# abcqmars/audio-visual-sepatation-in-visual-agnostic-situtation

Measured on AMD Instinct MI355X. Metric: mixtures/sec (train step, 2-src MUSIC shape), higher is better.
Workload: dtype f32; 1 GPU; full HIP path, AV train step: 2-source mix, batch 64/GPU (BASELINE configs[2] shape), 65535-sample waveforms -> HIP STFT 1022/256 -> 256x256 log-freq tiles, 3x224^2 frames/source, unet7+hidsep(sig)+resnet18dilated, BCE, SGD; f32 arithmetic; visual trunk on this library (no MIOpen kernel in the step); global_batch=64, parallelism=dp1

## Files before the change

### audio-visual-sepatation-in-visual-agnostic-situtation_amd/csrc/ops.hip

```cpp
#include "common.h"
#include "warp_coords.h"
#include <string.h>
#include <stdio.h>

__global__ __launch_bounds__(256) void channel_stats_kernel(const float* __restrict__ x, int N, int C, int HW,
                                                            double* __restrict__ stats) {
  const int c = blockIdx.x;
  const long long total = (long long)N * HW;
  const long long per = (total + gridDim.y - 1) / gridDim.y;
  const long long beg = per * blockIdx.y, end = min(total, beg + per);
  float s = 0.f, q = 0.f;
  double ds = 0.0, dq = 0.0;
  int cnt = 0;
  for (long long i = beg + threadIdx.x; i < end; i += 256) {
    int n = (int)(i / HW), hw = (int)(i % HW);
    float v = x[((long long)n * C + c) * HW + hw];
    s += v;
    q += v * v;
    if (++cnt == 64) { ds += s; dq += q; s = q = 0.f; cnt = 0; }
  }
  ds += s;
  dq += q;
  block_stats_add(ds, dq, c, C, stats);
}
// ... 857 lines not shown
      for (int s = 0; s < S; ++s) {
        float d = 1.f;
        if (act == AVSEP_ACT_SIGMOID) d = p[s] * (1.f - p[s]);
        else if (act == AVSEP_ACT_TANH) d = 1.f - p[s] * p[s];
        else if (act == AVSEP_ACT_RELU) d = l[s] > 0.f ? 1.f : 0.f;
        dlogits[((long long)b * S + s) * FT + i] = g[s] * d;
      }
    }
  }
}

extern "C" int avsep_mask_loss_bwd(const float* logits, const float* gt, const float* weight, int64_t w_target_stride,
                                   const float* coef, int32_t B, int32_t S, int32_t FT, int32_t act, int32_t loss,
                                   float* dlogits, avsep_stream_t stream) {
  if (!logits || !gt || !coef || !dlogits || B <= 0 || B > 65535 || S < 1 || S > MAXS || FT <= 0) return AVSEP_ERR_ARG;
  if (loss < 0 || loss > 2) return AVSEP_ERR_ARG;
  int gx = min(cdiv(FT, 1024), 64);
  hipLaunchKernelGGL(mask_loss_bwd_kernel, dim3(gx, B), dim3(256), 0, (hipStream_t)stream, logits, gt, weight,
                     (long long)w_target_stride, coef, B, S, FT, act, loss, dlogits);
  AVSEP_LAUNCH_CHECK();
  return AVSEP_OK;
}

__global__ __launch_bounds__(256) void maxpool_fwd_kernel(const float* __restrict__ x, const float* __restrict__ scale,
                                                          const float* __restrict__ shift, int act, int C, int NC, int H,
                                                          int W, int Ho, int Wo, float* __restrict__ y,
                                                          int* __restrict__ idx) {
  const long long total = (long long)NC * Ho * Wo;
  for (long long i = (long long)blockIdx.x * 256 + threadIdx.x; i < total; i += (long long)gridDim.x * 256) {
    int wo = (int)(i % Wo), ho = (int)((i / Wo) % Ho);
    long long nc = i / ((long long)Wo * Ho);
    const int c = (int)(nc % C);
    const float sc = scale ? scale[c] : 1.f, sh = scale ? shift[c] : 0.f;
    const float* p = x + nc * H * W;
    float best = -INFINITY;
    int bi = -1;
    for (int kh = 0; kh < 3; ++kh) {
      int h = ho * 2 - 1 + kh;
      if ((unsigned)h >= (unsigned)H) continue;
      for (int kw = 0; kw < 3; ++kw) {
        int w = wo * 2 - 1 + kw;
        if ((unsigned)w >= (unsigned)W) continue;
        float v = act_apply(fmaf(p[h * W + w], sc, sh), act);
        if (v > best || bi < 0) { best = v; bi = h * W + w; }
      }
    }
    y[i] = best;
    if (idx) idx[i] = bi;
  }
}
__global__ __launch_bounds__(256) void maxpool_fwd4_kernel(const float* __restrict__ x, const float* __restrict__ scale,
                                                           const float* __restrict__ shift, int act, int C, int H, int W,
                                                           int Ho, int Wo, float* __restrict__ y, int* __restrict__ idx) {
  const int nc = blockIdx.y, c = nc % C, Wq = Wo >> 2;
  const int t = blockIdx.x * 256 + threadIdx.x;
  if (t >= Ho * Wq) return;
  const int ho = t / Wq, q = t - ho * Wq;
  const float sc = scale ? scale[c] : 1.f, sh = scale ? shift[c] : 0.f, slope = act_slope(act);
  const float* p = x + (long long)nc * H * W;
  float best[4] = {-INFINITY, -INFINITY, -INFINITY, -INFINITY};
  int bi[4] = {-1, -1, -1, -1};
#pragma unroll
  for (int kh = 0; kh < 3; ++kh) {
    const int h = 2 * ho - 1 + kh;
    if ((unsigned)h >= (unsigned)H) continue;
    const float* row = p + h * W + 8 * q;
    const f32x4 a = *reinterpret_cast<const f32x4*>(row), b = *reinterpret_cast<const f32x4*>(row + 4);
    float v[9];
    v[0] = q > 0 ? row[-1] : 0.f;
    v[1] = a.x; v[2] = a.y; v[3] = a.z; v[4] = a.w; v[5] = b.x; v[6] = b.y; v[7] = b.z; v[8] = b.w;
#pragma unroll
    for (int k = 0; k < 9; ++k) v[k] = act_by_slope(fmaf(v[k], sc, sh), slope);
#pragma unroll
    for (int j = 0; j < 4; ++j)
#pragma unroll
      for (int kw = 0; kw < 3; ++kw) {
        const int k = 2 * j + kw;
        if (k == 0 && q == 0) continue;
        if (v[k] > best[j] || bi[j] < 0) { best[j] = v[k]; bi[j] = h * W + 8 * q - 1 + k; }
      }
  }
  const long long o = ((long long)nc * Ho + ho) * Wo + 4 * q;
  *reinterpret_cast<f32x4*>(y + o) = f32x4{best[0], best[1], best[2], best[3]};
  if (idx) *reinterpret_cast<int4*>(idx + o) = make_int4(bi[0], bi[1], bi[2], bi[3]);
}

enum { MAXPOOL_FWD_4, MAXPOOL_FWD_GENERIC };
static GluePlan maxpool_fwd_plan(int C, long long NC, int H, int W) {
  if (NC <= 0 || NC > 0x7fffffffLL || H <= 0 || W <= 0 || C <= 0 || NC % C) return glue_refused();
  int Ho = (H + 2 - 3) / 2 + 1, Wo = (W + 2 - 3) / 2 + 1;
  if ((W & 7) == 0 && (H & 1) == 0 && NC <= 65535 && (long long)H * W < 0x7fffffffLL)
    return GluePlan{MAXPOOL_FWD_4, dim3(cdiv(Ho * (Wo >> 2), 256), (unsigned)NC)};
  long long total = NC * Ho * Wo;
  return GluePlan{MAXPOOL_FWD_GENERIC, dim3((int)min((total + 255) / 256, (long long)65536))};
}
extern "C" int avsep_maxpool3x3s2_fwd(const float* x, const float* scale, const float* shift, int32_t act, int32_t C,
                                      int32_t NC, int32_t H, int32_t W, float* y, int32_t* idx, avsep_stream_t stream) {
  const GluePlan pl = maxpool_fwd_plan(C, NC, H, W);
  if (!x || !y || pl.refused()) return AVSEP_ERR_ARG;
  if ((scale == nullptr) != (shift == nullptr)) return AVSEP_ERR_ARG;
  int Ho = (H + 2 - 3) / 2 + 1, Wo = (W + 2 - 3) / 2 + 1;
  switch (pl.form) {
    case MAXPOOL_FWD_4:
      hipLaunchKernelGGL(maxpool_fwd4_kernel, pl.grid, dim3(256), 0, (hipStream_t)stream, x, scale, shift, act,
                         C, H, W, Ho, Wo, y, idx);
      break;
    case MAXPOOL_FWD_GENERIC:
      hipLaunchKernelGGL(maxpool_fwd_kernel, pl.grid, dim3(256), 0,
                         (hipStream_t)stream, x, scale, shift, act, C, NC, H, W, Ho, Wo, y, idx);
      break;
  }
  AVSEP_LAUNCH_CHECK();
  return AVSEP_OK;
}

__global__ __launch_bounds__(256) void maxpool_bwd_kernel(const float* __restrict__ dy, const int* __restrict__ idx, int NC,
                                                          int H, int W, int Ho, int Wo, float* __restrict__ dx) {
  const long long total = (long long)NC * H * W;
  for (long long i = (long long)blockIdx.x * 256 + threadIdx.x; i < total; i += (long long)gridDim.x * 256) {
    int w = (int)(i % W), h = (int)((i / W) % H);
    long long nc = i / ((long long)W * H);
    int self = h * W + w;
    float s = 0.f;
    for (int ho = h / 2; ho <= (h + 1) / 2 && ho < Ho; ++ho)
      for (int wo = w / 2; wo <= (w + 1) / 2 && wo < Wo; ++wo) {
        long long o = (nc * Ho + ho) * Wo + wo;
        if (idx[o] == self) s += dy[o];
      }
    dx[i] = s;
  }
}
static GluePlan maxpool_bwd_plan(long long NC, int H, int W) {
  if (NC <= 0 || NC > 0x7fffffffLL || H <= 0 || W <= 0) return glue_refused();
  long long total = NC * H * W;
  return GluePlan{0, dim3((int)min((total + 255) / 256, (long long)65536))};
}
// ... 191 lines not shown
                                               const float* shift, const float* pqr, int32_t N, int32_t C, int32_t H, int32_t W,
                                               float* dy, avsep_stream_t stream) {
  const GluePlan pl = maxpool_bn_relu_bwd_apply_plan(N, C, H, W);
  if (!g || !idx || !y || !scale || !shift || !pqr || !dy || pl.refused()) return AVSEP_ERR_ARG;
  const int Ho = (H + 2 - 3) / 2 + 1, Wo = (W + 2 - 3) / 2 + 1;
  switch (pl.form) {
    case POOL_BWD_APPLY_4:
      hipLaunchKernelGGL(maxpool_bn_relu_bwd_apply4_kernel, pl.grid, dim3(256), 0, (hipStream_t)stream, g, idx, y, scale,
                         shift, pqr, C, H, W, Ho, Wo, dy);
      break;
    case POOL_BWD_APPLY_PAIR:
      hipLaunchKernelGGL(maxpool_bn_relu_bwd_apply_kernel, pl.grid, dim3(256), 0, (hipStream_t)stream, g, idx, y, scale,
                         shift, pqr, C, H, W, Ho, Wo, dy);
      break;
    case POOL_BWD_APPLY_1:
      hipLaunchKernelGGL(maxpool_bn_relu_bwd_apply1_kernel, pl.grid, dim3(256), 0,
                         (hipStream_t)stream, g, idx, y, scale, shift, pqr, C, N * C, H, W, Ho, Wo, dy);
      break;
  }
  AVSEP_LAUNCH_CHECK();
  return AVSEP_OK;
}

__global__ __launch_bounds__(256) void temporal_mean_fwd_kernel(const float* __restrict__ x, int B, int T, long long CHW,
                                                                float* __restrict__ y) {
  const long long total = (long long)B * CHW;
  for (long long i = (long long)blockIdx.x * 256 + threadIdx.x; i < total; i += (long long)gridDim.x * 256) {
    long long b = i / CHW, r = i % CHW;
    float s = 0.f;
    for (int t = 0; t < T; ++t) s += x[(b * T + t) * CHW + r];
    y[i] = s / (float)T;
  }
}
static GluePlan flat_plan(long long total, long long cap) {
  return GluePlan{0, dim3((int)min((total + 255) / 256, cap))};
}
static GluePlan temporal_mean_plan(int B, int T, long long CHW, bool bwd) {
  if (B <= 0 || T <= 0 || CHW <= 0 || CHW > 0x7fffffffLL) return glue_refused();
  return flat_plan(bwd ? (long long)B * T * CHW : (long long)B * CHW, 65536);
}
extern "C" int avsep_temporal_mean_fwd(const float* x, int32_t B, int32_t T, int32_t CHW, float* y,
                                       avsep_stream_t stream) {
  const GluePlan pl = temporal_mean_plan(B, T, CHW, false);
  if (!x || !y || pl.refused()) return AVSEP_ERR_ARG;
  hipLaunchKernelGGL(temporal_mean_fwd_kernel, pl.grid, dim3(256), 0,
                     (hipStream_t)stream, x, B, T, (long long)CHW, y);
// ... 183 lines not shown
    atomicAdd(&sums[r * 3 + 2], sh[8] + sh[9] + sh[10] + sh[11]);
  }
}
extern "C" int avsep_sdr_sums(const float* est, const float* ref, int32_t R, int32_t L, int64_t est_stride,
                              int64_t ref_stride, double* sums, avsep_stream_t stream) {
  if (!est || !ref || !sums || R <= 0 || R > 65535 || L <= 0) return AVSEP_ERR_ARG;
  hipLaunchKernelGGL(sdr_sums_kernel, dim3(min(cdiv(L, 2048), 64), R), dim3(256), 0, (hipStream_t)stream, est, ref, L,
                     (long long)est_stride, (long long)ref_stride, sums);
  AVSEP_LAUNCH_CHECK();
  return AVSEP_OK;
}

static const GluePlanRow ops_glue_rows[] = {
    {"channel_stats", {"chunks"}, [](int N, int C, int H, int W, int) { return channel_stats_plan(N, C, (long long)H * W); }},
    {"bn_bwd_apply", {"vec4", "scalar"}, [](int N, int C, int H, int W, int) { return bn_bwd_apply_plan(N, C, (long long)H * W); }},
    {"affine_act", {"vec4", "scalar"}, [](int N, int C, int H, int W, int) { return affine_act_plan(N, C, (long long)H * W); }},
    {"affine_act_bwd", {"v4", "v1"}, [](int N, int C, int H, int W, int) { return affine_act_bwd_plan(N, C, (long long)H * W); }},
    {"relu_up2x_fwd", {"pair", "fwd4", "generic"}, [](int N, int C, int H, int W, int aux) { return relu_up2x_fwd_plan(N, C, H, W, aux != 0); }},
    {"relu_up2x_bwd", {"sweep,planes", "sweep", "tile"}, [](int N, int C, int H, int W, int aux) { return relu_up2x_bwd_plan(N, C, H, W, aux != 0); }},
    {"maxpool_fwd", {"fwd4", "generic"}, [](int N, int C, int H, int W, int) { return maxpool_fwd_plan(C, (long long)N * C, H, W); }},
    {"maxpool_bwd", {"gather"}, [](int N, int C, int H, int W, int) { return maxpool_bwd_plan((long long)N * C, H, W); }},
    {"maxpool_bn_relu_bwd_stats", {"plane"}, [](int N, int C, int H, int W, int) { return maxpool_bn_relu_bwd_stats_plan(N, C, H, W); }},
    {"maxpool_bn_relu_bwd_apply", {"apply4", "pair", "apply1"}, [](int N, int C, int H, int W, int) { return maxpool_bn_relu_bwd_apply_plan(N, C, H, W); }},
    {"space_to_depth2", {"planes"}, [](int N, int C, int H, int W, int Cp) { return space_to_depth2_plan(N, C, H, W, Cp); }},
    {"temporal_mean_fwd", {"flat"}, [](int B, int C, int H, int W, int T) { return temporal_mean_plan(B, T, (long long)C * H * W, false); }},
    {"temporal_mean_bwd", {"flat"}, [](int B, int C, int H, int W, int T) { return temporal_mean_plan(B, T, (long long)C * H * W, true); }},
    {"sgd", {"flat"}, [](int N, int C, int H, int W, int) { return flat_plan((long long)N * C * ((long long)H * W), 16384); }},
};

extern "C" int avsep_glue_plan(const char* op, int32_t N, int32_t C, int32_t H, int32_t W, int32_t aux, char* form, size_t cap,
                               int32_t grid[3]) {
  if (!op || !form || !grid || cap < 32 || N <= 0 || C <= 0 || H <= 0 || W <= 0 || aux < 0) return AVSEP_ERR_ARG;
  int counts[2] = {(int)(sizeof(ops_glue_rows) / sizeof(ops_glue_rows[0])), 0};
  const GluePlanRow* const tables[2] = {ops_glue_rows, b16_glue_rows(&counts[1])};
  for (int t = 0; t < 2; ++t)
    for (const GluePlanRow* r = tables[t]; r < tables[t] + counts[t]; ++r) {
      if (strcmp(op, r->op)) continue;
      const GluePlan p = r->plan(N, C, H, W, aux);
      if (p.refused()) return AVSEP_ERR_ARG;
      snprintf(form, cap, "%s", r->forms[p.form]);
      grid[0] = (int32_t)p.grid.x; grid[1] = (int32_t)p.grid.y; grid[2] = (int32_t)p.grid.z;
      return AVSEP_OK;
    }
  return AVSEP_ERR_ARG;
}

// ... 12 lines not shown
```

### audio-visual-sepatation-in-visual-agnostic-situtation_amd/kernels.py

```python
import ctypes as C
import os

import numpy as np
import torch

from . import lib
from .lib import ConvDesc, CatDesc, call, ptr


def _f32(shape, like):
    return torch.empty(shape, dtype=torch.float32, device=like.device)


FMT_F32, FMT_B16 = 0, 1


def is_b16(t):
    return t is not None and t.dtype == torch.bfloat16


def fmt_of(t):
    return FMT_B16 if is_b16(t) else FMT_F32


# ... 1235 lines not shown
        g, g2 = to_b16(g), to_b16(g2)
        call("avsep_b16_maxpool_bn_relu_bwd", ptr(g), ptr(g2), ptr(idx), ptr(y), ptr(bnrow[0]), ptr(bnrow[1]), ptr(bnrow[2]),
             ptr(bnrow[3]), None, N, Cc, H, W, ptr(bstats), None, 0)
        return
    assert g2 is None
    call("avsep_maxpool_bn_relu_bwd_stats", ptr(to_f32(g)), ptr(idx), ptr(y), ptr(bnrow[0]), ptr(bnrow[1]), ptr(bnrow[2]), ptr(bnrow[3]),
         N, Cc, H, W, ptr(bstats))


def maxpool_bn_relu_bwd_apply(g, idx, y, bnrow, pqr, g2=None, out_f32=False):
    N, Cc, H, W = dims(y)
    if is_b16(y):
        g, g2 = to_b16(g), to_b16(g2)
        dy = _f32((N, Cc, H, W), y) if out_f32 else torch.empty_like(y)
        call("avsep_b16_maxpool_bn_relu_bwd", ptr(g), ptr(g2), ptr(idx), ptr(y), ptr(bnrow[0]), ptr(bnrow[1]), None, None, ptr(pqr),
             N, Cc, H, W, None, ptr(dy), int(out_f32))
        return dy
    dy = torch.empty_like(y)
    assert g2 is None
    call("avsep_maxpool_bn_relu_bwd_apply", ptr(to_f32(g)), ptr(idx), ptr(y), ptr(bnrow[0]), ptr(bnrow[1]), ptr(pqr), N, Cc, H, W, ptr(dy))
    return dy


MISI_MAX_SOURCES = 8
MISI_MAX_GROUPS = 8


class Stft:

    def __init__(self, device, n_fft=1022, hop=256, pad_mode="reflect"):
        self.n_fft, self.hop, self.reflect = n_fft, hop, int(pad_mode == "reflect")
        L = lib.load()
        with torch.cuda.device(device):
            self.fwd_basis = torch.empty((L.avsep_stft_basis_floats(n_fft, 0),), dtype=torch.float32, device=device)
            self.inv_basis = torch.empty((L.avsep_stft_basis_floats(n_fft, 1),), dtype=torch.float32, device=device)
            call("avsep_stft_basis", n_fft, ptr(self.fwd_basis), ptr(self.inv_basis))

    def stft(self, wav, want_phase=True):
        R, Ln = wav.shape
        bins, frames = self.n_fft // 2 + 1, 1 + Ln // self.hop
        nbytes = lib.load().avsep_stft_workspace_bytes(R, Ln, self.n_fft, self.hop)
        ws = torch.empty((nbytes // 4,), dtype=torch.float32, device=wav.device)
        mag = _f32((R, bins, frames), wav)
        phase = _f32((R, bins, frames), wav) if want_phase else None
        call("avsep_stft_mag", ptr(wav), R, Ln, self.n_fft, self.hop, self.reflect, ptr(self.fwd_basis), ptr(mag),
             ptr(phase), ptr(ws), nbytes)
# ... 41 lines not shown
```

### audio-visual-sepatation-in-visual-agnostic-situtation_amd/lib.py

```python
import ctypes as C
import os

import torch

_HERE = os.path.dirname(os.path.abspath(__file__))
LIB_PATH = os.path.join(_HERE, "libavsep_gfx950.so")

ACT_NONE, ACT_RELU, ACT_LRELU02, ACT_SIGMOID, ACT_TANH, ACT_SOFTMAX2 = range(6)
ACT_BY_NAME = {"no": ACT_NONE, "relu": ACT_RELU, "sigmoid": ACT_SIGMOID, "tanh": ACT_TANH,
               "softmax": ACT_SOFTMAX2}
LOSS_BY_NAME = {"bce": 0, "l1": 1, "l2": 2}
ATT_BY_NAME = {"cos": 0, "sig": 1}
ALGO_NO = {"winograd": 1, "winograd_wgrad": 2, "flat": 4, "misc_patch": 8, "bf16_kernels": 16, "smallci_wgrad": 32, "winograd4": 64}


class AvsepError(RuntimeError):
    pass


class ConvDesc(C.Structure):
    _fields_ = [(n, C.c_int32) for n in
                "N Cin H W Cout Ho Wo KH KW stride pad dil C0 act0 act1 up2x prec plan_n xfmt yfmt dyfmt dxfmt algo tune".split()] + \
               [(n, C.c_void_p) for n in "x0 x1 scale0 shift0 scale1 shift1".split()]

# ... 28 lines not shown
_CD, _KD = C.POINTER(ConvDesc), C.POINTER(CatDesc)
_L = C.c_int64

SIGNATURES = {
    "avsep_version": (C.c_int, []),
    "avsep_arch": (C.c_char_p, []),
    "avsep_strerror": (C.c_char_p, [C.c_int]),
    "avsep_glue_plan": (C.c_int, [C.c_char_p, _I, _I, _I, _I, _I, C.c_char_p, _Z, C.POINTER(C.c_int32)]),
    "avsep_conv_packed_floats": (_Z, [_CD, C.c_int]),
    "avsep_conv_pack_weights": (C.c_int, [_CD, _P, _P, C.c_int, _P]),
    "avsep_conv_io_formats": (C.c_int, [_CD, _I, C.POINTER(C.c_int32), C.POINTER(C.c_int32)]),
    "avsep_conv2d_fwd_workspace_bytes": (_Z, [_CD]),
    "avsep_conv2d_fwd": (C.c_int, [_CD, _P, _P, _P, _P, _P, _Z, _P]),
    "avsep_conv2d_dgrad_workspace_bytes": (_Z, [_CD]),
    "avsep_conv2d_dgrad": (C.c_int, [_CD, _P, _P, _P, _P, _Z, _P]),
    "avsep_conv2d_dgrad_act_fused": (C.c_int32, [_CD]),
    "avsep_conv2d_dgrad_act": (C.c_int, [_CD, _P, _P, C.POINTER(ActBwd), _P, _P, _Z, _P]),
    "avsep_conv2d_head_applicable": (C.c_int32, [_CD]),
    "avsep_conv_kernel_name": (C.c_char_p, [_CD, _I, _I]),
    "avsep_conv_kernel_variant": (C.c_int, [_CD, _I, _I, C.c_char_p, _Z]),
    "avsep_space_to_depth2": (C.c_int, [_P, _I, _I, _I, _I, _I, _P, _P]),
    "avsep_maxpool_bn_relu_bwd_stats": (C.c_int, [_P, _P, _P, _P, _P, _P, _P, _I, _I, _I, _I, _P, _P]),
    "avsep_maxpool_bn_relu_bwd_apply": (C.c_int, [_P, _P, _P, _P, _P, _P, _I, _I, _I, _I, _P, _P]),
    "avsep_attmodel_infer_fwd": (C.c_int, [_P, _P, _I, _I, _I, _I, _I, _P, _P, _P, _P]),
    "avsep_attmodel_infer_bwd": (C.c_int, [_P, _P, _P, _P, _P, _P, _I, _I, _I, _I, _I, _P, _P, _P]),
    "avsep_conv2d_dgrad_up2x_workspace_bytes": (_Z, [_CD]),
    "avsep_conv2d_dgrad_up2x": (C.c_int, [_CD, _P, _P, _P, _P, _P, _P, _P, _I, _P, _Z, _P]),
    "avsep_conv2d_wgrad_workspace_bytes": (_Z, [_CD]),
    "avsep_conv2d_wgrad": (C.c_int, [_CD, _P, _P, _P, _P, _Z, _P]),
    "avsep_channel_stats": (C.c_int, [_P, _I, _I, _I, _P, _P]),
    "avsep_bn_finalize": (C.c_int, [_P, _D, _P, _P, _P, _P, _F, _F, _I, _I, _P, _P, _P, _P, _P, _I, _P]),
    "avsep_bn_bwd_coeffs": (C.c_int, [_P, _D, _P, _P, _P, _I, _P, _P, _P, _P]),
    "avsep_bn_bwd_apply": (C.c_int, [_P, _P, _P, _I, _I, _I, _P, _P]),
    "avsep_affine_act": (C.c_int, [_P, _P, _P, _P, _P, _P, _I, _I, _I, _I, _P, _P]),
    "avsep_affine_act_bwd": (C.c_int, [_P, _P, _P, _P, _P, _P, _P, _P, _P, _P, _P, _I, _I, _I, _I, _P, _P, _P]),
    "avsep_relu_up2x_fwd": (C.c_int, [_KD, _P, _P]),
    "avsep_relu_up2x_bwd": (C.c_int, [_KD, _P, _P, _P, _P, _P, _P, _I, _P]),
    "avsep_prepare": (C.c_int, [_P, _P, _I, _I, _I, _I, _I, _I, _I, _I, _P, _P, _P, _P, _P, _P]),
    "avsep_warp": (C.c_int, [_P, _I, _I, _I, _I, _I, _I, _P, _P]),
    "avsep_window_prepare": (C.c_int, [_P, _I, _I, _P, _I, _I, _I, _P, _P, _P]),
    "avsep_window_agreement": (C.c_int, [_P, _P, _I, _I, _I, _I, _P, _P]),
    "avsep_mask_stitch": (C.c_int, [_P, _P, _P, _P, _I, _I, _I, _I, _I, _I, _I, _I, _F, _P, _P, _P]),
    "avsep_window_reduce": (C.c_int, [_P, _P, _I, _I, C.c_int64, _I, _P, _P]),
    "avsep_mwf_workspace_bytes": (_Z, [_I, _I, _I, _I]),
    "avsep_mwf_cov": (C.c_int, [_P, _P, _I, _I, _I, _I, _I, _P, _P, _Z, _P]),
    "avsep_mwf_apply": (C.c_int, [_P, _P, _P, _P, _I, _I, _I, _I, _F, _P, _P, _P]),
# ... 124 lines not shown
```

### audio-visual-sepatation-in-visual-agnostic-situtation_amd/models/vision_hip.py

```python
import torch

from .. import kernels as K
from .. import lib
from ..lib import ACT_NONE, ACT_RELU
from .audio_net import ParamGrads, _bn_back, _bn_run


def _geom(conv):
    k, s, p, d = conv.kernel_size, conv.stride, conv.padding, conv.dilation
    if k[0] != k[1] or s[0] != s[1] or p[0] != p[1] or d[0] != d[1]:
        raise lib.AvsepError("the HIP visual trunk needs square conv geometry")
    return k[0], s[0], p[0], d[0]


def _w(conv):
    return conv.weight.detach().contiguous()


def _conv(src, conv, aff=None):
    k, s, p, d = _geom(conv)
    if aff is None:
        return K.Conv(src, conv.out_channels, k, s, p, d)
    return K.Conv(src, conv.out_channels, k, s, p, d, sc0=aff[0], sh0=aff[1], act0=ACT_RELU)


def _conv_bn(src, conv, bn, training, aff=None):
    cv = _conv(src, conv, aff)
    st = K.zeros_stats(conv.out_channels, src) if training else None
    y = cv.fwd(cv.pack(_w(conv), 0), None, st)
    return cv, y, _bn_run(bn, st, K.per_channel(y), training, src)


def blocks_of(features):
    return [b for i in (4, 5, 6, 7) for b in features[i]]


def param_list(net):
    return list(net.features.parameters()) + list(net.fc.parameters())


_S2D_INDEX = {}


def _stem_s2d_weight(w):
    Co, Cc = w.shape[:2]
    key = (Cc, w.device)
    if key not in _S2D_INDEX:
        idx = torch.zeros((16, 4, 4), dtype=torch.long)
        ok = torch.zeros((16, 4, 4), dtype=torch.bool)
        for q in range(4 * Cc):
            c, dy, dx = q % Cc, (q // Cc) >> 1, (q // Cc) & 1
            for a in range(4):
                for b in range(4):
                    kh, kw = 2 * a + dy - 1, 2 * b + dx - 1
                    if 0 <= kh <= 6 and 0 <= kw <= 6:
                        idx[q, a, b], ok[q, a, b] = (c * 7 + kh) * 7 + kw, True
        _S2D_INDEX[key] = (idx.to(w.device).reshape(-1), ok.to(w.device).reshape(1, 16, 4, 4))
    idx, ok = _S2D_INDEX[key]
    return (w.reshape(Co, -1)[:, idx].reshape(Co, 16, 4, 4) * ok).contiguous()


def _stem_s2d_weight_grad(dw2, Cc):
    Co = dw2.shape[0]
    key = ("inv", Cc, dw2.device)
    if key not in _S2D_INDEX:
        inv = torch.zeros((Cc, 7, 7), dtype=torch.long)
        for q in range(4 * Cc):
            c, dy, dx = q % Cc, (q // Cc) >> 1, (q // Cc) & 1
            for a in range(4):
                for b in range(4):
                    kh, kw = 2 * a + dy - 1, 2 * b + dx - 1
                    if 0 <= kh <= 6 and 0 <= kw <= 6:
                        inv[c, kh, kw] = (q * 4 + a) * 4 + b
        _S2D_INDEX[key] = inv.to(dw2.device).reshape(-1)
    return dw2.reshape(Co, -1)[:, _S2D_INDEX[key]].reshape(Co, Cc, 7, 7)


def _stem_is_s2d(conv, x):
    return (conv.kernel_size == (7, 7) and conv.stride == (2, 2) and conv.padding == (3, 3) and conv.dilation == (1, 1)
            and conv.in_channels <= 4 and x.shape[2] % 2 == 0 and x.shape[3] % 2 == 0)


def stem_forward(f, x, training):
    S = {"x": x}
    if _stem_is_s2d(f[0], x):
        S["cv0"] = _conv(x, f[0])
        cs = K.Conv(K.space_to_depth2(x), f[0].out_channels, 4, 1, 0)
        S["cs"] = cs
        st = K.zeros_stats(f[0].out_channels, x) if training else None
        S["y0"] = cs.fwd(cs.pack(_stem_s2d_weight(_w(f[0])), 0), None, st)
        S["bn0"] = _bn_run(f[1], st, K.per_channel(S["y0"]), training, x)
    else:
        S["cv0"], S["y0"], S["bn0"] = _conv_bn(x, f[0], f[1], training)
    z, S["idx"] = K.maxpool3x3s2(S["y0"], S["bn0"][0], S["bn0"][1], ACT_RELU)
    return S, z


def block_forward(blk, z, training):
    R = {"mod": blk, "z": z}
    R["cv1"], R["y1"], R["bn1"] = _conv_bn(z, blk.conv1, blk.bn1, training)
    if K.get_precision() == "f32":
        a1 = K.affine_act(R["y1"], R["bn1"][0], R["bn1"][1], None, ACT_RELU)
        R["cv2"], R["y2"], R["bn2"] = _conv_bn(a1, blk.conv2, blk.bn2, training)
    else:
        R["cv2"], R["y2"], R["bn2"] = _conv_bn(R["y1"], blk.conv2, blk.bn2, training, aff=R["bn1"])
    if blk.downsample is not None:
        R["cvd"], R["yd"], R["bnd"] = _conv_bn(z, blk.downsample[0], blk.downsample[1], training)
        out = K.affine_act(R["y2"], R["bn2"][0], R["bn2"][1], R["yd"], ACT_RELU, R["bnd"][0], R["bnd"][1])
    else:
        out = K.affine_act(R["y2"], R["bn2"][0], R["bn2"][1], R["z"], ACT_RELU)
    return R, out


def fc_forward(fc, z):
    cvf = _conv(z, fc)
    bias = fc.bias.detach() if fc.bias is not None else None
    return cvf, cvf.fwd(cvf.pack(_w(fc), 0), bias, None, out_b16=False)
# ... 36 lines not shown
        pqr1 = _bn_back(grads, blk.bn1, bn1, bst1, K.per_channel(R["y1"]))
        del dy2
    else:
        da = R["cv2"].dgrad(R["cv2"].pack(_w(blk.conv2), 1), dy2)
        del dy2
        da, pqr1 = _relu_bn_back(grads, da, R["y1"], R["bn1"], blk.bn1)
    da = K.bn_bwd_apply_(da, R["y1"], pqr1)
    grads.wgrad(R["cv1"], blk.conv1.weight, da)
    dz = R["cv1"].dgrad(R["cv1"].pack(_w(blk.conv1), 1), da)
    del da
    if ds:
        bst = K.zeros_stats(K.channels(g), g)
        g = K.affine_act_bwd_(g, R["yd"], None, None, None, None, bnd[2], bnd[3], ACT_NONE, bst, stats_only=True)
        pqrd = _bn_back(grads, blk.downsample[1], bnd, bst, K.per_channel(g))
        g = K.bn_bwd_apply_(g, R["yd"], pqrd)
        grads.wgrad(R["cvd"], blk.downsample[0].weight, g)
        return dz, R["cvd"].dgrad(R["cvd"].pack(_w(blk.downsample[0]), 1), g)
    return dz, g


def stem_backward(f, S, g, grads, g2=None):
    y0, bn0 = S["y0"], S["bn0"]
    g = g.contiguous()
    if g2 is not None and not K.is_b16(y0):
        g = K.to_f32(g).add_(K.to_f32(g2))
        g2 = None
    bst = K.zeros_stats(K.channels(y0), y0)
    K.maxpool_bn_relu_bwd_stats(g, S["idx"], y0, bn0, bst, g2)
    pqr0 = _bn_back(grads, f[1], bn0, bst, K.per_channel(y0))
    cs = S.get("cs")
    if cs is not None and K.is_b16(y0) and cs.io_formats(2)[0] == K.FMT_B16:
        dy0 = K.maxpool_bn_relu_bwd_apply(g, S["idx"], y0, bn0, pqr0, g2)
        dw2, _ = cs.wgrad(dy0)
        grads.add(f[0].weight, _stem_s2d_weight_grad(dw2, f[0].in_channels))
        return
    dy0 = K.maxpool_bn_relu_bwd_apply(g, S["idx"], y0, bn0, pqr0, g2, out_f32=True)
    grads.wgrad(S["cv0"], f[0].weight, dy0)


def trunk_backward(net, S, dout, grads):
    g = fc_backward(net.fc, S["cvf"], dout, grads)
    g2 = None
    for R in reversed(S["blocks"]):
        g, g2 = block_backward(R, g, grads, g2)
    stem_backward(net.features, S, g, grads, g2)


class _ResnetFn(torch.autograd.Function):
    @staticmethod
    def forward(ctx, net, x, *params):
# ... 18 lines not shown
```

### include/avsep.h

```cpp
#ifndef AVSEP_H
#define AVSEP_H
#include <stddef.h>
#include <stdint.h>

#ifdef __cplusplus
extern "C" {
#endif

#define AVSEP_OK 0
#define AVSEP_ERR_ARG (-1)
#define AVSEP_ERR_LAUNCH (-2)
#define AVSEP_ERR_WORKSPACE (-3)

#define AVSEP_ACT_NONE 0
#define AVSEP_ACT_RELU 1
#define AVSEP_ACT_LRELU02 2
#define AVSEP_ACT_SIGMOID 3
#define AVSEP_ACT_TANH 4
#define AVSEP_ACT_SOFTMAX2 5

#define AVSEP_PREC_F32 0
#define AVSEP_PREC_BF16 1

#define AVSEP_FMT_F32 0
// ... 163 lines not shown
size_t avsep_stft_basis_floats(int32_t n_fft, int32_t inverse);
int avsep_stft_basis(int32_t n_fft, float* fwd_basis, float* inv_basis, avsep_stream_t stream);
size_t avsep_stft_workspace_bytes(int32_t R, int32_t L, int32_t n_fft, int32_t hop);
int avsep_stft_mag(const float* wav, int32_t R, int32_t L, int32_t n_fft, int32_t hop,
                   int32_t reflect, const float* basis, float* mag, float* phase, void* workspace,
                   size_t workspace_bytes, avsep_stream_t stream);
size_t avsep_istft_workspace_bytes(int32_t R, int32_t n_fft, int32_t frames);
int avsep_istft(const float* mag, const float* phase, int32_t R, int32_t n_fft, int32_t hop,
                int32_t frames, const float* inv_basis, float* wav, int32_t out_len, void* workspace,
                size_t workspace_bytes, avsep_stream_t stream);

int avsep_maxpool3x3s2_fwd(const float* x, const float* scale, const float* shift, int32_t act, int32_t C,
                           int32_t NC, int32_t H, int32_t W, float* y, int32_t* idx, avsep_stream_t stream);
int avsep_maxpool3x3s2_bwd(const float* dy, const int32_t* idx, int32_t NC, int32_t H, int32_t W,
                           float* dx, avsep_stream_t stream);
int avsep_space_to_depth2(const float* x, int32_t N, int32_t C, int32_t H, int32_t W, int32_t Cp, float* xs,
                          avsep_stream_t stream);
int avsep_maxpool_bn_relu_bwd_stats(const float* g, const int32_t* idx, const float* y, const float* scale,
                                    const float* shift, const float* mean, const float* invstd, int32_t N, int32_t C,
                                    int32_t H, int32_t W, double* bstats, avsep_stream_t stream);
int avsep_maxpool_bn_relu_bwd_apply(const float* g, const int32_t* idx, const float* y, const float* scale,
                                    const float* shift, const float* pqr, int32_t N, int32_t C, int32_t H, int32_t W,
                                    float* dy, avsep_stream_t stream);
int avsep_temporal_mean_fwd(const float* x, int32_t B, int32_t T, int32_t CHW, float* y,
                            avsep_stream_t stream);
int avsep_temporal_mean_bwd(const float* dy, int32_t B, int32_t T, int32_t CHW, float* dx,
                            avsep_stream_t stream);
int avsep_sgd_momentum(float* p, const float* g, float* buf, size_t n, float lr, float momentum,
                       float weight_decay, float grad_scale, int32_t first, avsep_stream_t stream);
int avsep_innerprod_fwd(const float* img, const float* snd, const float* scale, const float* bias,
                        int32_t B, int32_t K, int32_t HW, float* z, avsep_stream_t stream);
int avsep_innerprod_nosum(const float* img, const float* snd, const float* scale, const float* bias,
                          int32_t B, int32_t K, int32_t HW, float* z, avsep_stream_t stream);
int avsep_innerprod_pixelwise(const float* imgs, const float* snd, const float* scale, const float* bias,
                              int32_t B, int32_t K, int32_t P, int32_t HW, float* z, avsep_stream_t stream);
int avsep_innerprod_bwd(const float* img, const float* snd, const float* scale, const float* dz,
                        int32_t B, int32_t K, int32_t HW, float* dsnd, float* r, avsep_stream_t stream);

int avsep_sdr_sums(const float* est, const float* ref, int32_t R, int32_t L, int64_t est_stride,
                   int64_t ref_stride, double* sums, avsep_stream_t stream);

int avsep_window_prepare(const float* mag, int32_t Fin, int32_t F, const int32_t* starts, int32_t K, int32_t Fout,
                         int32_t W, float* mag_w, float* log_mag_w, avsep_stream_t stream);
int avsep_window_agreement(const float* masks, const int32_t* starts, int32_t K, int32_t N, int32_t Fout, int32_t W,
                           double* D, avsep_stream_t stream);
int avsep_mask_stitch(const float* masks, const int32_t* starts, const int32_t* perm, const float* mag, int32_t K,
// ... 171 lines not shown
```

Before: 873.2 mixtures/s.

## Store uint8 tap indices and pre-activation max in stem maxpool for f32 backward

```diff
diff --git a/audio-visual-sepatation-in-visual-agnostic-situtation_amd/csrc/ops.hip b/audio-visual-sepatation-in-visual-agnostic-situtation_amd/csrc/ops.hip
--- a/audio-visual-sepatation-in-visual-agnostic-situtation_amd/csrc/ops.hip
+++ b/audio-visual-sepatation-in-visual-agnostic-situtation_amd/csrc/ops.hip
@@ -903,10 +903,12 @@
   return AVSEP_OK;
 }
 
+template <bool TAP>
 __global__ __launch_bounds__(256) void maxpool_fwd_kernel(const float* __restrict__ x, const float* __restrict__ scale,
                                                           const float* __restrict__ shift, int act, int C, int NC, int H,
                                                           int W, int Ho, int Wo, float* __restrict__ y,
-                                                          int* __restrict__ idx) {
+                                                          int* __restrict__ idx, unsigned char* __restrict__ tap,
+                                                          float* __restrict__ ymax) {
   const long long total = (long long)NC * Ho * Wo;
   for (long long i = (long long)blockIdx.x * 256 + threadIdx.x; i < total; i += (long long)gridDim.x * 256) {
     int wo = (int)(i % Wo), ho = (int)((i / Wo) % Ho);
@@ -914,7 +916,7 @@
     const int c = (int)(nc % C);
     const float sc = scale ? scale[c] : 1.f, sh = scale ? shift[c] : 0.f;
     const float* p = x + nc * H * W;
-    float best = -INFINITY;
+    float best = -INFINITY, braw = 0.f;
     int bi = -1;
     for (int kh = 0; kh < 3; ++kh) {
       int h = ho * 2 - 1 + kh;
@@ -922,24 +924,28 @@
       for (int kw = 0; kw < 3; ++kw) {
         int w = wo * 2 - 1 + kw;
         if ((unsigned)w >= (unsigned)W) continue;
-        float v = act_apply(fmaf(p[h * W + w], sc, sh), act);
-        if (v > best || bi < 0) { best = v; bi = h * W + w; }
+        const float raw = p[h * W + w];
+        float v = act_apply(fmaf(raw, sc, sh), act);
+        if (v > best || bi < 0) { best = v; bi = TAP ? kh * 3 + kw : h * W + w; braw = raw; }
       }
     }
     y[i] = best;
-    if (idx) idx[i] = bi;
-  }
-}
+    if constexpr (TAP) { tap[i] = (unsigned char)bi; ymax[i] = braw; }
+    else if (idx) idx[i] = bi;
+  }
+}
+template <bool TAP>
 __global__ __launch_bounds__(256) void maxpool_fwd4_kernel(const float* __restrict__ x, const float* __restrict__ scale,
                                                            const float* __restrict__ shift, int act, int C, int H, int W,
-                                                           int Ho, int Wo, float* __restrict__ y, int* __restrict__ idx) {
+                                                           int Ho, int Wo, float* __restrict__ y, int* __restrict__ idx,
+                                                           unsigned char* __restrict__ tap, float* __restrict__ ymax) {
   const int nc = blockIdx.y, c = nc % C, Wq = Wo >> 2;
   const int t = blockIdx.x * 256 + threadIdx.x;
   if (t >= Ho * Wq) return;
   const int ho = t / Wq, q = t - ho * Wq;
   const float sc = scale ? scale[c] : 1.f, sh = scale ? shift[c] : 0.f, slope = act_slope(act);
   const float* p = x + (long long)nc * H * W;
-  float best[4] = {-INFINITY, -INFINITY, -INFINITY, -INFINITY};
+  float best[4] = {-INFINITY, -INFINITY, -INFINITY, -INFINITY}, braw[4] = {0.f, 0.f, 0.f, 0.f};
   int bi[4] = {-1, -1, -1, -1};
 #pragma unroll
   for (int kh = 0; kh < 3; ++kh) {
@@ -947,23 +953,28 @@
     if ((unsigned)h >= (unsigned)H) continue;
     const float* row = p + h * W + 8 * q;
     const f32x4 a = *reinterpret_cast<const f32x4*>(row), b = *reinterpret_cast<const f32x4*>(row + 4);
-    float v[9];
-    v[0] = q > 0 ? row[-1] : 0.f;
-    v[1] = a.x; v[2] = a.y; v[3] = a.z; v[4] = a.w; v[5] = b.x; v[6] = b.y; v[7] = b.z; v[8] = b.w;
-#pragma unroll
-    for (int k = 0; k < 9; ++k) v[k] = act_by_slope(fmaf(v[k], sc, sh), slope);
+    float raw[9], v[9];
+    raw[0] = q > 0 ? row[-1] : 0.f;
+    raw[1] = a.x; raw[2] = a.y; raw[3] = a.z; raw[4] = a.w; raw[5] = b.x; raw[6] = b.y; raw[7] = b.z; raw[8] = b.w;
+#pragma unroll
+    for (int k = 0; k < 9; ++k) v[k] = act_by_slope(fmaf(raw[k], sc, sh), slope);
 #pragma unroll
     for (int j = 0; j < 4; ++j)
 #pragma unroll
       for (int kw = 0; kw < 3; ++kw) {
         const int k = 2 * j + kw;
         if (k == 0 && q == 0) continue;
-        if (v[k] > best[j] || bi[j] < 0) { best[j] = v[k]; bi[j] = h * W + 8 * q - 1 + k; }
+        if (v[k] > best[j] || bi[j] < 0) { best[j] = v[k]; bi[j] = TAP ? kh * 3 + kw : h * W + 8 * q - 1 + k; braw[j] = raw[k]; }
       }
   }
   const long long o = ((long long)nc * Ho + ho) * Wo + 4 * q;
   *reinterpret_cast<f32x4*>(y + o) = f32x4{best[0], best[1], best[2], best[3]};
-  if (idx) *reinterpret_cast<int4*>(idx + o) = make_int4(bi[0], bi[1], bi[2], bi[3]);
+  if constexpr (TAP) {
+    *reinterpret_cast<unsigned*>(tap + o) = (unsigned)bi[0] | (unsigned)bi[1] << 8 | (unsigned)bi[2] << 16 | (unsigned)bi[3] << 24;
+    *reinterpret_cast<f32x4*>(ymax + o) = f32x4{braw[0], braw[1], braw[2], braw[3]};
+  } else if (idx) {
+    *reinterpret_cast<int4*>(idx + o) = make_int4(bi[0], bi[1], bi[2], bi[3]);
+  }
 }
 
 enum { MAXPOOL_FWD_4, MAXPOOL_FWD_GENERIC };
@@ -975,24 +986,35 @@
   long long total = NC * Ho * Wo;
   return GluePlan{MAXPOOL_FWD_GENERIC, dim3((int)min((total + 255) / 256, (long long)65536))};
 }
-extern "C" int avsep_maxpool3x3s2_fwd(const float* x, const float* scale, const float* shift, int32_t act, int32_t C,
-                                      int32_t NC, int32_t H, int32_t W, float* y, int32_t* idx, avsep_stream_t stream) {
+template <bool TAP>
+static int maxpool_fwd_launch(const float* x, const float* scale, const float* shift, int act, int C, int NC, int H, int W,
+                              float* y, int* idx, unsigned char* tap, float* ymax, hipStream_t st) {
   const GluePlan pl = maxpool_fwd_plan(C, NC, H, W);
   if (!x || !y || pl.refused()) return AVSEP_ERR_ARG;
   if ((scale == nullptr) != (shift == nullptr)) return AVSEP_ERR_ARG;
   int Ho = (H + 2 - 3) / 2 + 1, Wo = (W + 2 - 3) / 2 + 1;
   switch (pl.form) {
     case MAXPOOL_FWD_4:
-      hipLaunchKernelGGL(maxpool_fwd4_kernel, pl.grid, dim3(256), 0, (hipStream_t)stream, x, scale, shift, act,
-                         C, H, W, Ho, Wo, y, idx);
+      hipLaunchKernelGGL(maxpool_fwd4_kernel<TAP>, pl.grid, dim3(256), 0, st, x, scale, shift, act, C, H, W, Ho, Wo, y, idx, tap,
+                         ymax);
       break;
     case MAXPOOL_FWD_GENERIC:
-      hipLaunchKernelGGL(maxpool_fwd_kernel, pl.grid, dim3(256), 0,
-                         (hipStream_t)stream, x, scale, shift, act, C, NC, H, W, Ho, Wo, y, idx);
+      hipLaunchKernelGGL(maxpool_fwd_kernel<TAP>, pl.grid, dim3(256), 0, st, x, scale, shift, act, C, NC, H, W, Ho, Wo, y, idx,
+                         tap, ymax);
       break;
   }
   AVSEP_LAUNCH_CHECK();
   return AVSEP_OK;
+}
+extern "C" int avsep_maxpool3x3s2_fwd(const float* x, const float* scale, const float* shift, int32_t act, int32_t C,
+                                      int32_t NC, int32_t H, int32_t W, float* y, int32_t* idx, avsep_stream_t stream) {
+  return maxpool_fwd_launch<false>(x, scale, shift, act, C, NC, H, W, y, idx, nullptr, nullptr, (hipStream_t)stream);
+}
+extern "C" int avsep_maxpool3x3s2_fwd_tap(const float* x, const float* scale, const float* shift, int32_t act, int32_t C,
+                                          int32_t NC, int32_t H, int32_t W, float* y, uint8_t* tap, float* ymax,
+                                          avsep_stream_t stream) {
+  if (!tap || !ymax) return AVSEP_ERR_ARG;
+  return maxpool_fwd_launch<true>(x, scale, shift, act, C, NC, H, W, y, nullptr, tap, ymax, (hipStream_t)stream);
 }
 
 __global__ __launch_bounds__(256) void maxpool_bwd_kernel(const float* __restrict__ dy, const int* __restrict__ idx, int NC,
@@ -1230,6 +1252,138 @@
   return AVSEP_OK;
 }
 
+__global__ __launch_bounds__(256) void maxpool_tap_bwd_stats_kernel(const float* __restrict__ g, const float* __restrict__ g2,
+                                                                    const float* __restrict__ ymax, const float* __restrict__ scale,
+                                                                    const float* __restrict__ shift, const float* __restrict__ mean,
+                                                                    const float* __restrict__ invstd, int C, int HoWo,
+                                                                    double* __restrict__ bstats) {
+  const int c = blockIdx.x, n = blockIdx.y;
+  const long long plane = ((long long)n * C + c) * HoWo;
+  const float sc = scale[c], sh = shift[c], mu = mean[c], is = invstd[c];
+  float s1 = 0.f, s2 = 0.f;
+  for (int o = threadIdx.x; o < HoWo; o += 256) {
+    const float yv = ymax[plane + o];
+    if (fmaf(yv, sc, sh) > 0.f) {
+      const float gv = g2 ? g[plane + o] + g2[plane + o] : g[plane + o];
+      s1 += gv;
+      s2 = fmaf(gv, (yv - mu) * is, s2);
+    }
+  }
+  block_stats_add((double)s1, (double)s2, c, C, bstats);
+}
+__global__ __launch_bounds__(256) void maxpool_tap_bwd_apply8_kernel(const float* __restrict__ g, const float* __restrict__ g2,
+                                                                     const unsigned char* __restrict__ tap, const float* __restrict__ y,
+                                                                     const float* __restrict__ scale, const float* __restrict__ shift,
+                                                                     const float* __restrict__ pqr, int C, int H, int W, int Ho, int Wo,
+                                                                     float* __restrict__ dy) {
+  const int nc = blockIdx.y, c = nc % C, We = W >> 3;
+  const float sc = scale[c], sh = shift[c], cp = pqr[c], cq = pqr[C + c], cr = pqr[2 * C + c];
+  const float* yp = y + (long long)nc * H * W;
+  float* dp = dy + (long long)nc * H * W;
+  const long long po = (long long)nc * Ho * Wo;
+  const float *gp = g + po, *g2p = g2 ? g2 + po : nullptr;
+  const unsigned char* tp = tap + po;
+  for (int i = blockIdx.x * 256 + threadIdx.x; i < H * We; i += gridDim.x * 256) {
+    const int h = i / We, j = i - h * We, self = h * W + 8 * j;
+    const f32x4 ya = *reinterpret_cast<const f32x4*>(yp + self), yb = *reinterpret_cast<const f32x4*>(yp + self + 4);
+    const float yv[8] = {ya.x, ya.y, ya.z, ya.w, yb.x, yb.y, yb.z, yb.w};
+    float s[8] = {0.f, 0.f, 0.f, 0.f, 0.f, 0.f, 0.f, 0.f};
+    const int ho0 = h >> 1, nho = (h & 1) && ho0 + 1 < Ho ? 2 : 1;
+    const bool fifth = 4 * j + 4 < Wo;
+    for (int a = 0; a < nho; ++a) {
+      const int o = (ho0 + a) * Wo + 4 * j;
+      const int t0 = (h - 2 * (ho0 + a) + 1) * 3;
+      f32x4 gq = *reinterpret_cast<const f32x4*>(gp + o);
+      if (g2p) gq += *reinterpret_cast<const f32x4*>(g2p + o);
+      const unsigned tq = *reinterpret_cast<const unsigned*>(tp + o);
+      float gv[5] = {gq.x, gq.y, gq.z, gq.w, 0.f};
+      int kv[5] = {(int)(tq & 255), (int)(tq >> 8 & 255), (int)(tq >> 16 & 255), (int)(tq >> 24), 255};
+      if (fifth) {
+        gv[4] = g2p ? gp[o + 4] + g2p[o + 4] : gp[o + 4];
+        kv[4] = tp[o + 4];
+      }
+#pragma unroll
+      for (int b = 0; b < 5; ++b)
+#pragma unroll
+        for (int kw = 0; kw < 3; ++kw) {
+          const int p = 2 * b - 1 + kw;
+          if (p >= 0 && p < 8 && kv[b] == t0 + kw) s[p] += gv[b];
+        }
+    }
+    float out[8];
+#pragma unroll
+    for (int k = 0; k < 8; ++k) {
+      const float sk = fmaf(yv[k], sc, sh) > 0.f ? s[k] : 0.f;
+      out[k] = fmaf(cp, sk, fmaf(cq, yv[k], cr));
+    }
+    *reinterpret_cast<f32x4*>(dp + self) = f32x4{out[0], out[1], out[2], out[3]};
+    *reinterpret_cast<f32x4*>(dp + self + 4) = f32x4{out[4], out[5], out[6], out[7]};
+  }
+}
+__global__ __launch_bounds__(256) void maxpool_tap_bwd_apply1_kernel(const float* __restrict__ g, const float* __restrict__ g2,
+                                                                     const unsigned char* __restrict__ tap, const float* __restrict__ y,
+                                                                     const float* __restrict__ scale, const float* __restrict__ shift,
+                                                                     const float* __restrict__ pqr, int C, int NC, int H, int W, int Ho,
+                                                                     int Wo, float* __restrict__ dy) {
+  const long long total = (long long)NC * H * W;
+  for (long long i = (long long)blockIdx.x * 256 + threadIdx.x; i < total; i += (long long)gridDim.x * 256) {
+    const int w = (int)(i % W), h = (int)((i / W) % H);
+    const long long nc = i / ((long long)W * H);
+    const int c = (int)(nc % C);
+    const float yv = y[i];
+    float s = 0.f;
+    if (fmaf(yv, scale[c], shift[c]) > 0.f) {
+      for (int ho = h / 2; ho <= (h + 1) / 2 && ho < Ho; ++ho)
+        for (int wo = w / 2; wo <= (w + 1) / 2 && wo < Wo; ++wo) {
+          const long long o = (nc * Ho + ho) * Wo + wo;
+          if (tap[o] == (h - 2 * ho + 1) * 3 + (w - 2 * wo + 1)) s += g2 ? g[o] + g2[o] : g[o];
+        }
+    }
+    dy[i] = fmaf(pqr[c], s, fmaf(pqr[C + c], yv, pqr[2 * C + c]));
+  }
+}
+enum { POOL_TAP_APPLY_8, POOL_TAP_APPLY_1 };
+static GluePlan maxpool_tap_bwd_apply_plan(int N, int C, int H, int W) {
+  if (N <= 0 || C <= 0 || H <= 0 || W <= 0) return glue_refused();
+  const long long total = (long long)N * C * H * W;
+  if ((W & 7) == 0 && (long long)N * C <= 65535 && (long long)H * W < 0x7fffffffLL) {
+    const int per = H * (W / 8), gx = (per + 255) / 256 < 64 ? (per + 255) / 256 : 64;
+    return GluePlan{POOL_TAP_APPLY_8, dim3(gx, N * C)};
+  }
+  return GluePlan{POOL_TAP_APPLY_1, dim3((int)min((total + 255) / 256, (long long)262144))};
+}
+extern "C" int avsep_maxpool_tap_bn_relu_bwd_stats(const float* g, const float* g2, const float* ymax, const float* scale,
+                                                   const float* shift, const float* mean, const float* invstd, int32_t N,
+                                                   int32_t C, int32_t H, int32_t W, double* bstats, avsep_stream_t stream) {
+  if (!g || !ymax || !scale || !shift || !mean || !invstd || !bstats) return AVSEP_ERR_ARG;
+  const GluePlan pl = maxpool_bn_relu_bwd_stats_plan(N, C, H, W);
+  if (pl.refused()) return AVSEP_ERR_ARG;
+  const int Ho = (H + 2 - 3) / 2 + 1, Wo = (W + 2 - 3) / 2 + 1;
+  hipLaunchKernelGGL(maxpool_tap_bwd_stats_kernel, pl.grid, dim3(256), 0, (hipStream_t)stream, g, g2, ymax, scale, shift, mean,
+                     invstd, C, Ho * Wo, bstats);
+  AVSEP_LAUNCH_CHECK();
+  return AVSEP_OK;
+}
+extern "C" int avsep_maxpool_tap_bn_relu_bwd_apply(const float* g, const float* g2, const uint8_t* tap, const float* y,
+                                                   const float* scale, const float* shift, const float* pqr, int32_t N,
+                                                   int32_t C, int32_t H, int32_t W, float* dy, avsep_stream_t stream) {
+  const GluePlan pl = maxpool_tap_bwd_apply_plan(N, C, H, W);
+  if (!g || !tap || !y || !scale || !shift || !pqr || !dy || pl.refused()) return AVSEP_ERR_ARG;
+  const int Ho = (H + 2 - 3) / 2 + 1, Wo = (W + 2 - 3) / 2 + 1;
+  switch (pl.form) {
+    case POOL_TAP_APPLY_8:
+      hipLaunchKernelGGL(maxpool_tap_bwd_apply8_kernel, pl.grid, dim3(256), 0, (hipStream_t)stream, g, g2, tap, y, scale, shift,
+                         pqr, C, H, W, Ho, Wo, dy);
+      break;
+    case POOL_TAP_APPLY_1:
+      hipLaunchKernelGGL(maxpool_tap_bwd_apply1_kernel, pl.grid, dim3(256), 0, (hipStream_t)stream, g, g2, tap, y, scale, shift,
+                         pqr, C, N * C, H, W, Ho, Wo, dy);
+      break;
+  }
+  AVSEP_LAUNCH_CHECK();
+  return AVSEP_OK;
+}
+
 __global__ __launch_bounds__(256) void temporal_mean_fwd_kernel(const float* __restrict__ x, int B, int T, long long CHW,
                                                                 float* __restrict__ y) {
   const long long total = (long long)B * CHW;
@@ -1459,6 +1613,9 @@
     {"maxpool_bwd", {"gather"}, [](int N, int C, int H, int W, int) { return maxpool_bwd_plan((long long)N * C, H, W); }},
     {"maxpool_bn_relu_bwd_stats", {"plane"}, [](int N, int C, int H, int W, int) { return maxpool_bn_relu_bwd_stats_plan(N, C, H, W); }},
     {"maxpool_bn_relu_bwd_apply", {"apply4", "pair", "apply1"}, [](int N, int C, int H, int W, int) { return maxpool_bn_relu_bwd_apply_plan(N, C, H, W); }},
+    {"maxpool_fwd_tap", {"fwd4", "generic"}, [](int N, int C, int H, int W, int) { return maxpool_fwd_plan(C, (long long)N * C, H, W); }},
+    {"maxpool_tap_bwd_stats", {"plane"}, [](int N, int C, int H, int W, int) { return maxpool_bn_relu_bwd_stats_plan(N, C, H, W); }},
+    {"maxpool_tap_bwd_apply", {"apply8", "apply1"}, [](int N, int C, int H, int W, int) { return maxpool_tap_bwd_apply_plan(N, C, H, W); }},
     {"space_to_depth2", {"planes"}, [](int N, int C, int H, int W, int Cp) { return space_to_depth2_plan(N, C, H, W, Cp); }},
     {"temporal_mean_fwd", {"flat"}, [](int B, int C, int H, int W, int T) { return temporal_mean_plan(B, T, (long long)C * H * W, false); }},
     {"temporal_mean_bwd", {"flat"}, [](int B, int C, int H, int W, int T) { return temporal_mean_plan(B, T, (long long)C * H * W, true); }},
diff --git a/audio-visual-sepatation-in-visual-agnostic-situtation_amd/kernels.py b/audio-visual-sepatation-in-visual-agnostic-situtation_amd/kernels.py
--- a/audio-visual-sepatation-in-visual-agnostic-situtation_amd/kernels.py
+++ b/audio-visual-sepatation-in-visual-agnostic-situtation_amd/kernels.py
@@ -1281,6 +1281,29 @@
     return dy
 
 
+def maxpool3x3s2_tap(x, scale=None, shift=None, act=0):
+    N, Cc, H, W = x.shape
+    Ho, Wo = out_size(H, 3, 2, 1, 1), out_size(W, 3, 2, 1, 1)
+    y, ymax = _f32((N, Cc, Ho, Wo), x), _f32((N, Cc, Ho, Wo), x)
+    tap = torch.empty((N, Cc, Ho, Wo), dtype=torch.uint8, device=x.device)
+    call("avsep_maxpool3x3s2_fwd_tap", ptr(x), ptr(scale), ptr(shift), act, Cc, N * Cc, H, W, ptr(y), ptr(tap), ptr(ymax))
+    return y, tap, ymax
+
+
+def maxpool_tap_bn_relu_bwd_stats(g, g2, ymax, H, W, bnrow, bstats):
+    N, Cc = ymax.shape[:2]
+    call("avsep_maxpool_tap_bn_relu_bwd_stats", ptr(g), ptr(g2), ptr(ymax), ptr(bnrow[0]), ptr(bnrow[1]), ptr(bnrow[2]),
+         ptr(bnrow[3]), N, Cc, H, W, ptr(bstats))
+
+
+def maxpool_tap_bn_relu_bwd_apply(g, g2, tap, y, bnrow, pqr):
+    N, Cc, H, W = y.shape
+    dy = torch.empty_like(y)
+    call("avsep_maxpool_tap_bn_relu_bwd_apply", ptr(g), ptr(g2), ptr(tap), ptr(y), ptr(bnrow[0]), ptr(bnrow[1]), ptr(pqr),
+         N, Cc, H, W, ptr(dy))
+    return dy
+
+
 MISI_MAX_SOURCES = 8
 MISI_MAX_GROUPS = 8
 
diff --git a/audio-visual-sepatation-in-visual-agnostic-situtation_amd/lib.py b/audio-visual-sepatation-in-visual-agnostic-situtation_amd/lib.py
--- a/audio-visual-sepatation-in-visual-agnostic-situtation_amd/lib.py
+++ b/audio-visual-sepatation-in-visual-agnostic-situtation_amd/lib.py
@@ -74,6 +74,9 @@
     "avsep_space_to_depth2": (C.c_int, [_P, _I, _I, _I, _I, _I, _P, _P]),
     "avsep_maxpool_bn_relu_bwd_stats": (C.c_int, [_P, _P, _P, _P, _P, _P, _P, _I, _I, _I, _I, _P, _P]),
     "avsep_maxpool_bn_relu_bwd_apply": (C.c_int, [_P, _P, _P, _P, _P, _P, _I, _I, _I, _I, _P, _P]),
+    "avsep_maxpool3x3s2_fwd_tap": (C.c_int, [_P, _P, _P, _I, _I, _I, _I, _I, _P, _P, _P, _P]),
+    "avsep_maxpool_tap_bn_relu_bwd_stats": (C.c_int, [_P, _P, _P, _P, _P, _P, _P, _I, _I, _I, _I, _P, _P]),
+    "avsep_maxpool_tap_bn_relu_bwd_apply": (C.c_int, [_P, _P, _P, _P, _P, _P, _P, _I, _I, _I, _I, _P, _P]),
     "avsep_attmodel_infer_fwd": (C.c_int, [_P, _P, _I, _I, _I, _I, _I, _P, _P, _P, _P]),
     "avsep_attmodel_infer_bwd": (C.c_int, [_P, _P, _P, _P, _P, _P, _I, _I, _I, _I, _I, _P, _P, _P]),
     "avsep_conv2d_dgrad_up2x_workspace_bytes": (_Z, [_CD]),
diff --git a/audio-visual-sepatation-in-visual-agnostic-situtation_amd/models/vision_hip.py b/audio-visual-sepatation-in-visual-agnostic-situtation_amd/models/vision_hip.py
--- a/audio-visual-sepatation-in-visual-agnostic-situtation_amd/models/vision_hip.py
+++ b/audio-visual-sepatation-in-visual-agnostic-situtation_amd/models/vision_hip.py
@@ -42,12 +42,12 @@
 _S2D_INDEX = {}
 
 
-def _stem_s2d_weight(w):
+def _stem_s2d_weight(w, cp=16):
     Co, Cc = w.shape[:2]
-    key = (Cc, w.device)
+    key = (Cc, cp, w.device)
     if key not in _S2D_INDEX:
-        idx = torch.zeros((16, 4, 4), dtype=torch.long)
-        ok = torch.zeros((16, 4, 4), dtype=torch.bool)
+        idx = torch.zeros((cp, 4, 4), dtype=torch.long)
+        ok = torch.zeros((cp, 4, 4), dtype=torch.bool)
         for q in range(4 * Cc):
             c, dy, dx = q % Cc, (q // Cc) >> 1, (q // Cc) & 1
             for a in range(4):
@@ -55,9 +55,9 @@
                     kh, kw = 2 * a + dy - 1, 2 * b + dx - 1
                     if 0 <= kh <= 6 and 0 <= kw <= 6:
                         idx[q, a, b], ok[q, a, b] = (c * 7 + kh) * 7 + kw, True
-        _S2D_INDEX[key] = (idx.to(w.device).reshape(-1), ok.to(w.device).reshape(1, 16, 4, 4))
+        _S2D_INDEX[key] = (idx.to(w.device).reshape(-1), ok.to(w.device).reshape(1, cp, 4, 4))
     idx, ok = _S2D_INDEX[key]
-    return (w.reshape(Co, -1)[:, idx].reshape(Co, 16, 4, 4) * ok).contiguous()
+    return (w.reshape(Co, -1)[:, idx].reshape(Co, cp, 4, 4) * ok).contiguous()
 
 
 def _stem_s2d_weight_grad(dw2, Cc):
@@ -85,14 +85,18 @@
     S = {"x": x}
     if _stem_is_s2d(f[0], x):
         S["cv0"] = _conv(x, f[0])
-        cs = K.Conv(K.space_to_depth2(x), f[0].out_channels, 4, 1, 0)
+        cp = 12 if K.get_precision() == "f32" and f[0].in_channels == 3 else 16
+        cs = K.Conv(K.space_to_depth2(x, cp), f[0].out_channels, 4, 1, 0)
         S["cs"] = cs
         st = K.zeros_stats(f[0].out_channels, x) if training else None
-        S["y0"] = cs.fwd(cs.pack(_stem_s2d_weight(_w(f[0])), 0), None, st)
+        S["y0"] = cs.fwd(cs.pack(_stem_s2d_weight(_w(f[0]), cp), 0), None, st)
         S["bn0"] = _bn_run(f[1], st, K.per_channel(S["y0"]), training, x)
     else:
         S["cv0"], S["y0"], S["bn0"] = _conv_bn(x, f[0], f[1], training)
-    z, S["idx"] = K.maxpool3x3s2(S["y0"], S["bn0"][0], S["bn0"][1], ACT_RELU)
+    if K.is_b16(S["y0"]):
+        z, S["idx"] = K.maxpool3x3s2(S["y0"], S["bn0"][0], S["bn0"][1], ACT_RELU)
+    else:
+        z, S["tap"], S["ymax"] = K.maxpool3x3s2_tap(S["y0"], S["bn0"][0], S["bn0"][1], ACT_RELU)
     return S, z
 
 
@@ -175,10 +179,14 @@
 def stem_backward(f, S, g, grads, g2=None):
     y0, bn0 = S["y0"], S["bn0"]
     g = g.contiguous()
-    if g2 is not None and not K.is_b16(y0):
-        g = K.to_f32(g).add_(K.to_f32(g2))
-        g2 = None
     bst = K.zeros_stats(K.channels(y0), y0)
+    if not K.is_b16(y0):
+        g, g2 = K.to_f32(g), (K.to_f32(g2).contiguous() if g2 is not None else None)
+        K.maxpool_tap_bn_relu_bwd_stats(g, g2, S["ymax"], y0.shape[2], y0.shape[3], bn0, bst)
+        pqr0 = _bn_back(grads, f[1], bn0, bst, K.per_channel(y0))
+        dy0 = K.maxpool_tap_bn_relu_bwd_apply(g, g2, S["tap"], y0, bn0, pqr0)
+        grads.wgrad(S["cv0"], f[0].weight, dy0)
+        return
     K.maxpool_bn_relu_bwd_stats(g, S["idx"], y0, bn0, bst, g2)
     pqr0 = _bn_back(grads, f[1], bn0, bst, K.per_channel(y0))
     cs = S.get("cs")
diff --git a/include/avsep.h b/include/avsep.h
--- a/include/avsep.h
+++ b/include/avsep.h
@@ -209,6 +209,15 @@
 int avsep_maxpool_bn_relu_bwd_apply(const float* g, const int32_t* idx, const float* y, const float* scale,
                                     const float* shift, const float* pqr, int32_t N, int32_t C, int32_t H, int32_t W,
                                     float* dy, avsep_stream_t stream);
+int avsep_maxpool3x3s2_fwd_tap(const float* x, const float* scale, const float* shift, int32_t act, int32_t C,
+                               int32_t NC, int32_t H, int32_t W, float* y, uint8_t* tap, float* ymax,
+                               avsep_stream_t stream);
+int avsep_maxpool_tap_bn_relu_bwd_stats(const float* g, const float* g2, const float* ymax, const float* scale,
+                                        const float* shift, const float* mean, const float* invstd, int32_t N, int32_t C,
+                                        int32_t H, int32_t W, double* bstats, avsep_stream_t stream);
+int avsep_maxpool_tap_bn_relu_bwd_apply(const float* g, const float* g2, const uint8_t* tap, const float* y,
+                                        const float* scale, const float* shift, const float* pqr, int32_t N, int32_t C,
+                                        int32_t H, int32_t W, float* dy, avsep_stream_t stream);
 int avsep_temporal_mean_fwd(const float* x, int32_t B, int32_t T, int32_t CHW, float* y,
                             avsep_stream_t stream);
 int avsep_temporal_mean_bwd(const float* dy, int32_t B, int32_t T, int32_t CHW, float* dx,
```

After: 881.7 mixtures/s, median of 6. Within noise of the previous version (+1.0%).
